# klae01/fft-conv-pytorch

Hardware: AMD Instinct MI355X
Metric: GSamples/s (output elems/s), forward fft_conv (higher is better)
Workload: dtype f32; 1 GPU; cfgA: 1D fft_conv B=32/GPU 8->8ch groups=1 spatial=[32768] kernel=[512] dilation=1 bias, fp32; tile=1024, buffer_sets=9, hip_graph=True, launches_per_graph=576, kernel_spectrum=cached per weight version (FFTConv module)

## Files before the change

### fft_conv_pytorch_amd/_native.py

```python
from __future__ import annotations

import collections
import ctypes
import os
import threading
from typing import Optional, Tuple

_HERE = os.path.dirname(os.path.abspath(__file__))
LIB_NAME = "libfftconv_amd.so"
LIB_PATH = os.environ.get("FFTCONV_LIB") or os.path.join(_HERE, LIB_NAME)

FC_OK, FC_ERR_INVALID, FC_ERR_UNSUPPORTED, FC_ERR_HIP = 0, 1, 2, 3
PAD_MODES = {"constant": 0, "zeros": 0, "reflect": 1, "replicate": 2, "circular": 3}
ABI_VERSION = 7

EXPORTS = (
    "fc_version", "fc_last_error", "fc_plan_create", "fc_plan_destroy", "fc_output_shape",
    "fc_kernel_spectrum_bytes", "fc_workspace_bytes", "fc_plan_tile", "fc_plan_layout", "fc_transform_kernel",
    "fc_forward", "fc_forward_stamped", "fc_wgrad1d_slices", "fc_wgrad1d", "fc_wgrad1d_db", "fc_wgrad1d_db_supported",
    "fc_debug_grid", "fc_wgrad_nd_plan_create", "fc_wgrad_nd", "fc_debug_route",
    "fc_long_geometry", "fc_long_plan_create", "fc_long_plan_destroy", "fc_long_plan_info", "fc_long_transform_kernel",
    "fc_long_forward", "fc_long_transform_kernel_io", "fc_long_forward_io",
    "fc_long_geometry_ext", "fc_long_plan_create_ext",
    "fc_long_geometry_kind", "fc_long_plan_create_kind", "fc_long_plan_kind",
    "fc_long_forward_lay",
    "fc_long_phases_geometry", "fc_long_phases_plan_create",
    "fc_long_decim_geometry", "fc_long_decim_plan_create",
    "fc_long_wgrad_geometry", "fc_long_wgrad_check_io", "fc_long_wgrad_plan_create", "fc_long_wgrad_plan_destroy",
    "fc_long_wgrad_plan_info", "fc_long_wgrad",
)

ROUTE_KINDS = ("f32_1d", "f32_nd", "f64_direct", "f64_fft_1d", "f64_fft_nd", "f64_fft_long")
ROUTE_WORDS = {
    "f32_1d": ("T", "ntiles", "pers_nb", "ph", "ph2", "slot_tiles", "nseg", "diag", "bd_gs", "wide", "dense",
               "chunk_launches", "accumulate", "n_ochunks", "pers_items"),
# ... 117 lines not shown
        lib.fc_wgrad1d_db.restype = i32
        lib.fc_wgrad1d_db_supported.argtypes = [ctypes.POINTER(FcDesc)]
        lib.fc_wgrad1d_db_supported.restype = i32
        lib.fc_wgrad_nd_plan_create.argtypes = [ctypes.POINTER(FcDesc), ctypes.POINTER(vp)]
        lib.fc_wgrad_nd_plan_create.restype = i32
        lib.fc_wgrad_nd.argtypes = [vp, vp, vp, vp, vp, vp, vp]
        lib.fc_wgrad_nd.restype = i32
        lib.fc_forward_stamped.argtypes = [vp, vp, vp, vp, vp, vp, vp, vp]
        lib.fc_forward_stamped.restype = i32
        lib.fc_plan_layout.argtypes = [vp, ctypes.POINTER(ctypes.c_int32 * 8)]
        lib.fc_plan_layout.restype = i32
        lib.fc_debug_grid.argtypes = [vp]
        lib.fc_debug_grid.restype = ctypes.c_longlong
        lib.fc_debug_route.argtypes = [vp, ctypes.POINTER(ctypes.c_int32 * 16)]
        lib.fc_debug_route.restype = i32
        i64x8 = ctypes.POINTER(ctypes.c_int64 * 8)
        lib.fc_long_geometry.argtypes = [ctypes.POINTER(FcLongDesc), i64x8]
        lib.fc_long_geometry.restype = i32
        lib.fc_long_plan_create.argtypes = [ctypes.POINTER(FcLongDesc), ctypes.POINTER(vp)]
        lib.fc_long_plan_create.restype = i32
        lib.fc_long_plan_destroy.argtypes = [vp]
        lib.fc_long_plan_destroy.restype = None
        lib.fc_long_plan_info.argtypes = [vp, i64x8]
        lib.fc_long_plan_info.restype = i32
        lib.fc_long_transform_kernel.argtypes = [vp, vp, vp, vp, vp]
        lib.fc_long_transform_kernel.restype = i32
        lib.fc_long_forward.argtypes = [vp, vp, vp, vp, vp, vp, vp]
        lib.fc_long_forward.restype = i32
        lib.fc_long_transform_kernel_io.argtypes = [vp, vp, i32, vp, vp, vp]
        lib.fc_long_transform_kernel_io.restype = i32
# ... 92 lines not shown

    def run(self, x_ptr: int, dy_ptr: int, dw_ptr: int, spectrum_ptr: int, workspace_ptr: Optional[int], stream: int):
        st = self._lib.fc_wgrad_nd(self._h, x_ptr, dy_ptr, dw_ptr, spectrum_ptr, workspace_ptr, stream)
        if st != FC_OK:
            _raise(self._lib, st)

    def __del__(self):
        try:
            if getattr(self, "_h", None):
                self._lib.fc_plan_destroy(self._h)
                self._h = None
        except Exception:
            pass


def read_route(lib, handle) -> dict:
    words = (ctypes.c_int32 * 16)()
    st = lib.fc_debug_route(handle, ctypes.byref(words))
    if st != FC_OK:
        _raise(lib, st)
    kind = ROUTE_KINDS[words[0]]
    route = {"kind": kind}
    route.update({name: int(words[1 + i]) for i, name in enumerate(ROUTE_WORDS[kind])})
    return route


def _raise(lib, status: int):
    msg = lib.fc_last_error().decode("utf-8", "replace")
    if status == FC_ERR_INVALID:
        raise ValueError(msg)
# ... 52 lines not shown
                workspace_ptr: Optional[int], stream: int):
        if self._stamps is not None:
            st = self._lib.fc_forward_stamped(self._h, x_ptr, w_hat_ptr, bias_ptr, y_ptr, workspace_ptr, stream,
                                              self._stamps)
        else:
            st = self._lib.fc_forward(self._h, x_ptr, w_hat_ptr, bias_ptr, y_ptr, workspace_ptr, stream)
        if st != FC_OK:
            _raise(self._lib, st)

    def debug_set_stamps(self, ptr: Optional[int]):
        self._stamps = ptr

    def debug_grid(self) -> int:
        return int(self._lib.fc_debug_grid(self._h))

    def __del__(self):
        try:
            if getattr(self, "_h", None):
                self._lib.fc_plan_destroy(self._h)
                self._h = None
        except Exception:
            pass


def long_desc(key: Tuple) -> FcLongDesc:
    if len(key) not in (11, 15, 16):
        raise ValueError(f"a long-plan key has 11 words, 15 with (pad_mode, src_up, tap_dil, out_step), or 16 with those and "
                         f"the kind of a complex plan; got {len(key)}")
    d = FcLongDesc()
    (d.batch, d.in_channels, d.out_channels, d.groups, d.length, d.kernel, d.pad_left, d.pad_right, d.out_keep,
# ... 236 lines not shown
```

### fft_conv_pytorch_amd/csrc/conv1d_pers.hpp

```cpp
#pragma once
#include "conv1d_fused.hpp"

namespace fc {

struct WorkItem {
  int b0, nbc, tile, goc;
};

struct Conv1dPersArgs {
  Conv1dArgs c;
  const WorkItem* items;
  int n_items;
};

__device__ __forceinline__ void stamp_item(unsigned long long* buf, int item, int slot) {
  if (buf != nullptr && (threadIdx.x & 63) == 0)
    buf[((size_t)item * 16 + (threadIdx.x >> 6)) * 16 + slot] = __builtin_amdgcn_s_memrealtime();
}
__device__ __forceinline__ void stamp_clock(unsigned long long* buf, int item, int slot) {
  if (buf != nullptr && (threadIdx.x & 63) == 0)
    buf[((size_t)item * 16 + (threadIdx.x >> 6)) * 16 + slot] = __builtin_amdgcn_s_memtime();
}

namespace pers {
// ... 24 lines not shown
  constexpr int T = G::T;
  constexpr int NPI = CIB / 2;
  constexpr int NSEQ = NB * NPI;
  static_assert(NT == NSEQ * G::TS, "one thread slot per point group of every sequence");
  static_assert((T / 2) % NT == 0, "bin pairs divide evenly over the threads");
  static_assert(NPI % 2 == 0, "the spectrum pipeline alternates two register sets");
  static_assert(NB * CIB * 2 <= 64, "the self-paired bins are handled by one wave");
  constexpr int BP = (T / 2) / NT;
  constexpr int TWN = P * G::N2;
  extern __shared__ __attribute__((aligned(16))) f2 lds[];
  const Conv1dArgs& a = pa.c;
  const Io<IO> io(a.io);
  constexpr unsigned ES = Io<IO>::B;
  auto stampi = [&](int item, int slot) { if constexpr (STAMPS) stamp_item(a.stamps, item, slot); };
  auto stampc = [&](int item, int slot) { if constexpr (STAMPS) stamp_clock(a.stamps, item, slot); };
  const int nph = PHASES ? a.ph : 1;

  const int tid = threadIdx.x;
  const int sq = tid / G::TS;
  const int tseq = tid % G::TS;
  static_assert(G::TS <= 64 && (NPI * G::TS) % 64 == 0, "a batch slot is a whole number of wavefronts");
  const int wv = __builtin_amdgcn_readfirstlane(tid >> 6);
  const int nb = PH4 ? ((tid >> 5) & 1) : (PH2 ? 2 * (wv / NPI) + ((tid >> 5) & 1)
               : (BPAIR ? 2 * __builtin_amdgcn_readfirstlane(tid / (CIB * G::TS)) : __builtin_amdgcn_readfirstlane(tid / (NPI * G::TS))));
  const int pr = PH4 ? wv : (PH2 ? wv % NPI : (BPAIR ? sq % CIB : sq % NPI));
  f2* twl = lds;
  f2* zbuf = lds + TWN;
  f2* zseq = PH4 ? zbuf + (nb * 8 + pr) * G::LSEQ : zbuf + (nb * NPI + pr) * G::LSEQ;

  const PadMap pm = make_padmap(a.pad_mode, a.L);
  const BufRsrc twB = make_rsrc(a.twB, (unsigned)(S * P * 8));
  const size_t wgroup = (size_t)a.Cog_pad * (a.Cig_pad / 2) * (T / 2);

  auto fetch = [&](const WorkItem& wi, f2 (&v)[P]) {
    if constexpr (BPAIR) {
      const int g = wi.goc / a.n_ochunks;
      const int bA = a.slot_tiles ? wi.b0 : wi.b0 + nb, bB = a.slot_tiles ? bA : bA + 1;
      const int tA = a.slot_tiles ? wi.tile + nb : wi.tile, tB = a.slot_tiles ? tA + 1 : tA;
      const int bfirst = wi.b0, blast = a.slot_tiles ? bfirst : wi.b0 + wi.nbc - 1;
      const int posA = tA * a.V - a.pad + (SEG ? a.pos_shift : 0), posB = tB * a.V - a.pad + (SEG ? a.pos_shift : 0);
      const bool interior = (posA >= 0) && (posA + (T - 1) < a.L) && (posB >= 0) && (posB + (T - 1) < a.L);
      const auto* xbase = io_ptr<IO>(a.x) + ((size_t)bfirst * a.Cin + (size_t)g * a.Cig) * a.L;
      const BufRsrc xg = make_rsrc(xbase, (unsigned)(((size_t)(blast - bfirst) * a.Cin + a.Cig) * a.L * ES));
      const bool hasA = nb < wi.nbc && pr < a.Cig, hasB = nb + 1 < wi.nbc && pr < a.Cig;
      const unsigned roA = ((unsigned)(bA - bfirst) * (unsigned)a.Cin + (unsigned)pr) * (unsigned)a.L * ES;
      const unsigned roB = ((unsigned)(bB - bfirst) * (unsigned)a.Cin + (unsigned)pr) * (unsigned)a.L * ES;
      if (interior && hasB) {
        const unsigned v0 = roA + (unsigned)(posA + tseq) * ES, v1 = roB + (unsigned)(posB + tseq) * ES;
#pragma unroll
        for (int n1 = 0; n1 < P; ++n1) {
          v[n1].x = io.load(xg, v0, G::N2 * n1 * ES);
          v[n1].y = io.load(xg, v1, G::N2 * n1 * ES);
        }
      } else {
#pragma unroll
        for (int n1 = 0; n1 < P; ++n1) {
          v[n1].x = io.load(xg, padded_offset<ES>(roA, posA + G::N2 * n1 + tseq, a.L, a.pad, pm, hasA), 0);
          v[n1].y = io.load(xg, padded_offset<ES>(roB, posB + G::N2 * n1 + tseq, a.L, a.pad, pm, hasB), 0);
        }
      }
      return;
    }
    const int g = wi.goc / a.n_ochunks;
    const int vb = a.slot_tiles ? wi.b0 : wi.b0 + nb;
    const int tile = a.slot_tiles ? wi.tile + nb : wi.tile;
    const int bfirst = wi.b0 / nph, blast = a.slot_tiles ? bfirst : (wi.b0 + wi.nbc - 1) / nph;
    const int b = vb / nph, phase = vb - b * nph;
    const int pos0 = tile * a.V * nph + phase - a.pad + (SEG ? a.pos_shift : 0);
    const bool interior = (pos0 >= 0) && (pos0 + (T - 1) * nph < a.L);
    const bool act_in = nb < wi.nbc;
    const auto* xbase = io_ptr<IO>(a.x) + ((size_t)bfirst * a.Cin + (size_t)g * a.Cig) * a.L;
    const BufRsrc xg = make_rsrc(xbase, (unsigned)(((size_t)(blast - bfirst) * a.Cin + a.Cig) * a.L * ES));
    const int ci0 = 2 * pr;
    const bool has0 = act_in && ci0 < a.Cig && (!DIAG || g * CIB + ci0 < a.Cin);
    const bool has1 = act_in && ci0 + 1 < a.Cig && (!DIAG || g * CIB + ci0 + 1 < a.Cin);
    const unsigned ro0 = ((unsigned)(b - bfirst) * (unsigned)a.Cin + (unsigned)ci0) * (unsigned)a.L * ES;
    const unsigned ro1 = ro0 + (unsigned)a.L * ES;
    if constexpr (PH4) {
      const int bA = wi.b0 / nph, phA = wi.b0 - bA * nph;
      const int posA = wi.tile * a.V * nph + phA - a.pad;
      const bool all_in = (posA >= 0) && (posA + 3 + (T - 1) * nph < a.L);
      const bool chan = pr < a.Cig;
      const unsigned rA = ((unsigned)(bA - bfirst) * (unsigned)a.Cin + (unsigned)pr) * (unsigned)a.L * ES;
      const bool al16 = (((size_t)xbase | ((size_t)a.L * ES) | ((size_t)(unsigned)posA * ES)) & (4 * ES - 1)) == 0;
      if (all_in && al16) {
        const unsigned q0 = chan ? rA + (unsigned)(posA + (tid & 63) * nph) * ES : 0x80000000u;
        const unsigned step4 = 64u * ES * (unsigned)nph;
#pragma unroll
        for (int m = 0; m < P / 2; ++m) {
          const f4 q = io.load4(xg, q0, step4 * m);
          v[2 * m] = q.xy; v[2 * m + 1] = q.zw;
        }
        return;
      }
      const unsigned ro = ((unsigned)(bA - bfirst) * (unsigned)a.Cin + (unsigned)pr) * (unsigned)a.L * ES;
#pragma unroll
      for (int n1 = 0; n1 < P; ++n1) {
        const int pos = posA + 2 * nb + (G::N2 * n1 + tseq) * nph;
        v[n1].x = io.load(xg, padded_offset<ES>(ro, pos, a.L, a.pad, pm, chan), 0);
        v[n1].y = io.load(xg, padded_offset<ES>(ro, pos + 1, a.L, a.pad, pm, chan), 0);
      }
      return;
    }
    if constexpr (PH2) {
      const int vbA = wi.b0 + 2 * (wv / NPI), bA = vbA / nph, phA = vbA - bA * nph;
      const int posA = wi.tile * a.V * nph + phA - a.pad;
      const bool both_in = (posA >= 0) && (posA + 1 + (T - 1) * nph < a.L);
      if (both_in && __all(has1)) {
        const unsigned rA = ((unsigned)(bA - bfirst) * (unsigned)a.Cin + (unsigned)ci0) * (unsigned)a.L * ES;
        const unsigned q0 = rA + (unsigned)(posA + (tid & 63) * nph) * ES, q1 = q0 + (unsigned)a.L * ES;
        const unsigned step2 = 64u * ES * (unsigned)nph;
#pragma unroll
        for (int m = 0; m < P / 2; ++m) {
          f2 cx = io.load2(xg, q0, step2 * m), cy = io.load2(xg, q1, step2 * m);
          v[2 * m].x = cx.x; v[2 * m + 1].x = cx.y; v[2 * m].y = cy.x; v[2 * m + 1].y = cy.y;
        }
        return;
      }
    }
    if (interior && has1 && !PHASES) {
      const unsigned v0 = ro0 + (unsigned)(pos0 + tseq) * ES, v1 = ro1 + (unsigned)(pos0 + tseq) * ES;
#if FC_DIAG == 7
#pragma unroll
      for (int n1 = 0; n1 < P; ++n1) { v[n1] = mk2(1e-3f * n1, (float)tseq); asm volatile("" : "+v"(v[n1])); }
      (void)v0; (void)v1;
      return;
#endif
#pragma unroll
      for (int n1 = 0; n1 < P; ++n1) {
        v[n1].x = io.load(xg, v0, G::N2 * n1 * ES);
        v[n1].y = io.load(xg, v1, G::N2 * n1 * ES);
      }
    } else if (interior && has1) {
      const unsigned v0 = ro0 + (unsigned)(pos0 + tseq * nph) * ES, v1 = ro1 + (unsigned)(pos0 + tseq * nph) * ES;
      const unsigned step = (unsigned)(G::N2 * ES) * (unsigned)nph;
#pragma unroll
      for (int n1 = 0; n1 < P; ++n1) {
        v[n1].x = io.load(xg, v0, step * n1);
        v[n1].y = io.load(xg, v1, step * n1);
      }
    } else {
#pragma unroll
      for (int n1 = 0; n1 < P; ++n1) {
        const int pos = pos0 + (G::N2 * n1 + tseq) * nph;
        v[n1].x = io.load(xg, padded_offset<ES>(ro0, pos, a.L, a.pad, pm, has0), 0);
        v[n1].y = io.load(xg, padded_offset<ES>(ro1, pos, a.L, a.pad, pm, has1), 0);
      }
    }
  };

  auto fetch_finish = [&](const WorkItem& wi, f2 (&v)[P]) {
    if constexpr (PH4) {
      const int bA = wi.b0 / nph, phA = wi.b0 - bA * nph;
      const int posA = wi.tile * a.V * nph + phA - a.pad;
      const int bfirst = wi.b0 / nph;
      const auto* xbase = io_ptr<IO>(a.x) + ((size_t)bfirst * a.Cin + (size_t)(wi.goc / a.n_ochunks) * a.Cig) * a.L;
      const bool all_in = (posA >= 0) && (posA + 3 + (T - 1) * nph < a.L);
      const bool al16 = (((size_t)xbase | ((size_t)a.L * ES) | ((size_t)(unsigned)posA * ES)) & (4 * ES - 1)) == 0;
      if (all_in && al16) {
#pragma unroll
        for (int m = 0; m < P / 2; ++m) { swap_halves_c<0>(v[2 * m], v[2 * m + 1]); swap_halves_c<1>(v[2 * m], v[2 * m + 1]); }
      }
    }
    if constexpr (PH2) {
      const bool has1 = nb < wi.nbc && 2 * pr + 1 < a.Cig;
      const int vbA = wi.b0 + 2 * (wv / NPI), bA = vbA / nph, phA = vbA - bA * nph;
      const int posA = wi.tile * a.V * nph + phA - a.pad;
      const bool both_in = (posA >= 0) && (posA + 1 + (T - 1) * nph < a.L);
      if (both_in && __all(has1)) {
#pragma unroll
        for (int m = 0; m < P / 2; ++m) { swap_halves_c<0>(v[2 * m], v[2 * m + 1]); swap_halves_c<1>(v[2 * m], v[2 * m + 1]); }
      }
    }
  };

  auto run = [&](const WorkItem& wi, int it, f2 (&v)[P], bool more, const WorkItem& wnext, f2 (&vnext)[P]) {
    const int g = wi.goc / a.n_ochunks, oc = wi.goc % a.n_ochunks;
    const bool act_in = PH4 ? true : nb < wi.nbc;
    const BufRsrc wg = DIAG ? make_rsrc(a.wspec + (size_t)g * NPI * (T / 2), (unsigned)(NPI * (T / 2) * 16))
                            : make_rsrc(a.wspec + (size_t)g * wgroup, (unsigned)(wgroup * 16));
    stampi(it, 0);
    stampc(it, 12);
    const int cg0 = g * a.Cog + oc * a.cob + ((PH4 || BPAIR) ? pr : 2 * pr);
    const bool ok0 = !DIAG || cg0 < a.Cout, ok1 = !BPAIR && (!DIAG || cg0 + 1 < a.Cout);
    const BufRsrc brs = make_rsrc(a.bias, a.bias ? (unsigned)a.Cout * 4u : 0u);
    float bias0 = buf_load_f32(brs, ok0 ? (unsigned)cg0 * 4u : 0xFFFFFFFFu, 0);
    float bias1 = BPAIR ? 0.f : buf_load_f32(brs, ok1 ? (unsigned)(cg0 + 1) * 4u : 0xFFFFFFFFu, 0);
    if (STAMPS && a.stamps) { asm volatile("s_waitcnt vmcnt(0)" ::: "memory"); stampi(it, 1); }
    if (act_in) {
      fetch_finish(wi, v);
      passA_fft_twiddle_store_lds<G, -1>(v, zseq, tseq, twl);
      stampi(it, 2);
// ... 342 lines not shown
#pragma unroll
        for (int p = 0; p < NPI; ++p) {
          acc = fmaf(2.f * sbz[p].x, (tid & 1) ? sbw[p].y : sbw[p].x, acc);
          acc = fmaf(2.f * sbz[p].y, (tid & 1) ? sbw[p].w : sbw[p].z, acc);
        }
        float* dstf = reinterpret_cast<float*>(zbuf + (sb_b * NPI + (sb_o >> 1)) * G::LSEQ + G::nat(sb_f)) + (sb_o & 1);
        *dstf = acc;
      }
    }
    }
    stampi(it, 6);
#if FC_DIAG != 5
    __syncthreads();
#endif
    stampi(it, 7);
    asm volatile("" : "+v"(bias0), "+v"(bias1));
    if (more) fetch(wnext, vnext);
    if (act_in) {
      nat_load<G>(v, zseq, tseq);
      seq_sync<G>();
      passA_fft_twiddle_store_lds<G, +1>(v, zseq, tseq, twl);
      stampi(it, 8);
      seq_sync<G>();
      stampi(it, 9);
      passB_load<G>(v, zseq, tseq);
      const int j = passB_compute<G, +1>(v, tseq, twB);
      if (more) {
#pragma unroll
        for (int n1 = 0; n1 < P; ++n1) asm volatile("" : "+v"(vnext[n1]));
      }
      const int o1 = tseq >> G::LGS;
// ... 165 lines not shown
                io.store(v[2 * m + 1].y + bias1, yr, (w1 + ES) | dB, step2 * m);
              }
            });
          }
        });
      } else {
        const int ystep = P * nph;
#pragma unroll
        for (int k = 0; k < P; ++k)
          if (nbase + P * k < limit) { y0[ystep * k] = io.out(v[k].x + bias0); y1[ystep * k] = io.out(v[k].y + bias1); }
      }
    }
    stampi(it, 10);
    if (STAMPS && a.stamps) { asm volatile("s_waitcnt vmcnt(0)" ::: "memory"); stampi(it, 11); stampc(it, 13); }
    seq_sync<G>();
  };

  const int it0 = blockIdx.x, it1 = blockIdx.x + gridDim.x;
  const bool two = it1 < pa.n_items;
  const WorkItem w0 = pa.items[it0];
  const WorkItem w1 = pa.items[two ? it1 : it0];
  f2 va[P], vb[P];
  fetch(w0, va);
  copy_table_to_lds<TWN, NT>(twl, a.twA, tid);
  __syncthreads();
  run(w0, it0, va, two, w1, vb);
  if (two) run(w1, it1, vb, false, w1, va);
}

}
```

### fft_conv_pytorch_amd/csrc/fc_api.cpp

```cpp
#include <hip/hip_runtime.h>

#include <cmath>
#include <cstdarg>
#include <cstdio>
#include <cstdlib>
#include <cstring>
#include <map>
#include <memory>
#include <mutex>
#include <string>
#include <vector>

#include "fc_plan.h"

namespace {

thread_local std::string g_err;
std::mutex g_tw_mutex;
std::map<std::pair<int, int>, fc::Twiddles> g_tw;

}

namespace fc {

// ... 291 lines not shown
  switch (p.kind) {
    case PlanKind::F32_1D:
      if (p.f1d.pers_nb) return (long long)p.f1d.pers_items * 16;
      return (long long)p.d.batch * p.ntiles * p.n_ochunks * p.G;
    case PlanKind::F32_ND:
      if (p.fnd.planes) {
        const long long ncol = p.fnd.planes == 1 ? (long long)fc::kPlCols * p.fnd.nxt * p.fnd.nyt : p.fnd.Fxt;
        return (long long)p.d.batch * p.ntiles * (p.fnd.Cog_pad / p.fnd.cob) * p.d.groups * ((ncol / 16 + 7) / 8) * 8;
      } else {
        const long long ncol = p.nd == 2 ? p.fnd.Fxt : (long long)p.fnd.Fxt * p.fnd.tm->T * p.fnd.nyt;
        return (long long)p.d.batch * p.ntiles * (p.fnd.Cog_pad / p.fnd.cob) * p.d.groups * ((ncol + 7) / 8) * 8;
      }
    default:
      return 0;
  }
}

int fc_debug_route(const fc_plan* plan, int32_t route[16]) {
  if (!plan || !route) return fail(FC_ERR_INVALID, "null argument");
  const fc_plan& p = *plan;
  for (int i = 0; i < 16; ++i) route[i] = 0;
  route[0] = (int32_t)p.kind;
  switch (p.kind) {
    case PlanKind::F32_1D: {
      const int32_t w[] = {p.tile->T, p.ntiles, p.f1d.pers_nb, p.f1d.ph, p.f1d.ph2, p.f1d.slot_tiles, p.f1d.nseg,
                           p.f1d.diag, p.f1d.bd_gs, p.f1d.wide, p.f1d.dense, p.f1d.chunk_launches, p.accumulate,
                           p.n_ochunks, p.f1d.pers_items};
      for (int i = 0; i < 15; ++i) route[1 + i] = w[i];
      break;
    }
// ... 106 lines not shown
```

### fft_conv_pytorch_amd/csrc/fc_plan.h

```cpp
#pragma once
#include <hip/hip_runtime.h>

#include <cstdint>
#include <cstring>

#include "fc_internal.h"
#include "fftconv_amd.h"

namespace fc {

int fail(int code, const char* fmt, ...);

#define FC_HIP(expr)                                                                         \
  do {                                                                                       \
    hipError_t e_ = (expr);                                                                  \
    if (e_ != hipSuccess) return ::fc::fail(FC_ERR_HIP, "%s: %s", #expr, hipGetErrorString(e_)); \
  } while (0)

#define FC_HIP_SETUP(expr)                                                               \
  do {                                                                                   \
    hipError_t e_ = (expr);                                                              \
    if (e_ != hipSuccess) {                                                              \
      const char* name_ = hipGetErrorName(e_);                                           \
      (void)hipGetLastError();                                                           \
// ... 5 lines not shown
    }                                                                                    \
  } while (0)

const TileImpl* const* all_tiles(int* n);
const TileImpl* find_tile(int T);

struct Twiddles {
  f2* twA = nullptr;
  f2* twB = nullptr;
};
int get_twiddles(const TileImpl* t, Twiddles* out);
int find_twiddles(const TileImpl* t, Twiddles* out);

int current_device_cus(int* cus_out);
int64_t round_up(int64_t v, int64_t m);

enum class PlanKind {
  F32_1D,
  F32_ND,
  F64_DIRECT,
  F64_FFT_1D,
  F64_FFT_ND,
  F64_FFT_LONG,
};

}

struct fc_plan {
  fc_desc d;
  fc::PlanKind kind;
// ... 93 lines not shown
```

### fft_conv_pytorch_amd/csrc/fft_engine.hpp

```cpp
#pragma once
#include <hip/hip_runtime.h>
#include <type_traits>

#ifndef FC_DIAG
#define FC_DIAG 0
#endif

namespace fc {

typedef float f2 __attribute__((ext_vector_type(2)));
typedef float f4 __attribute__((ext_vector_type(4)));

__device__ __forceinline__ f2 pkfma(f2 a, f2 b, f2 c) { return __builtin_elementwise_fma(a, b, c); }
__device__ __forceinline__ f2 mk2(float x, float y) { f2 r; r.x = x; r.y = y; return r; }
__device__ __forceinline__ f2 add_mi(f2 a, f2 b) {
  f2 d; asm("v_pk_add_f32 %0, %1, %2 op_sel:[0,1] op_sel_hi:[1,0] neg_hi:[0,1]" : "=v"(d) : "v"(a), "v"(b)); return d;
}
__device__ __forceinline__ f2 add_pi(f2 a, f2 b) {
  f2 d; asm("v_pk_add_f32 %0, %1, %2 op_sel:[0,1] op_sel_hi:[1,0] neg_lo:[0,1]" : "=v"(d) : "v"(a), "v"(b)); return d;
}
__device__ __forceinline__ f2 add_conj(f2 a, f2 b) {
  f2 d; asm("v_pk_add_f32 %0, %1, %2 neg_hi:[0,1]" : "=v"(d) : "v"(a), "v"(b)); return d;
}
__device__ __forceinline__ f2 sub_conj_divi(f2 a, f2 b) {
// ... 217 lines not shown
constexpr int IO_F32 = 0, IO_H16 = 1;
constexpr int IO_CODE_F16 = 2, IO_CODE_BF16 = 3;
constexpr bool io_is_h16(int code) { return code == IO_CODE_F16 || code == IO_CODE_BF16; }
template <int IO>
struct Io;
template <>
struct Io<IO_F32> {
  using T = float;
  static constexpr unsigned B = 4;
  __device__ __forceinline__ explicit Io(int) {}
  __device__ __forceinline__ float in(float v) const { return v; }
  __device__ __forceinline__ float out(float v) const { return v; }
  __device__ __forceinline__ float load(BufRsrc r, unsigned voff, unsigned soff) const { return buf_load_f32(r, voff, soff); }
  __device__ __forceinline__ f2 load2(BufRsrc r, unsigned voff, unsigned soff) const { return buf_load_f32x2(r, voff, soff); }
  __device__ __forceinline__ f4 load4(BufRsrc r, unsigned voff, unsigned soff) const { return buf_load_f32x4(r, voff, soff); }
  __device__ __forceinline__ void store(float v, BufRsrc r, unsigned voff, unsigned soff) const { buf_store_f32(v, r, voff, soff); }
  __device__ __forceinline__ void store2(f2 v, BufRsrc r, unsigned voff, unsigned soff) const { buf_store_f32x2(v, r, voff, soff); }
  __device__ __forceinline__ void store4(f4 v, BufRsrc r, unsigned voff, unsigned soff) const {
    u32x4 d;
    d.x = __float_as_uint(v.x); d.y = __float_as_uint(v.y); d.z = __float_as_uint(v.z); d.w = __float_as_uint(v.w);
    __builtin_amdgcn_raw_buffer_store_b128(d, r, voff, soff, 0);
  }
};
template <>
struct Io<IO_H16> {
  using T = unsigned short;
  static constexpr unsigned B = 2;
  bool bf;
  __device__ __forceinline__ explicit Io(int code) : bf(code == IO_CODE_BF16) {}
  __device__ __forceinline__ float in(unsigned h) const {
// ... 7 lines not shown
  }
  __device__ __forceinline__ unsigned pack(float lo, float hi) const {
    const bf16x2 b = {(__bf16)lo, (__bf16)hi};
    const f16x2 h = {(_Float16)lo, (_Float16)hi};
    return bf ? __builtin_bit_cast(unsigned, b) : __builtin_bit_cast(unsigned, h);
  }
  __device__ __forceinline__ float load(BufRsrc r, unsigned voff, unsigned soff) const {
    return in(__builtin_amdgcn_raw_buffer_load_b16(r, voff, soff, 0));
  }
  __device__ __forceinline__ f2 load2(BufRsrc r, unsigned voff, unsigned soff) const {
    const unsigned w = __builtin_amdgcn_raw_buffer_load_b32(r, voff, soff, 0);
    return mk2(in(w), in(w >> 16));
  }
  __device__ __forceinline__ f4 load4(BufRsrc r, unsigned voff, unsigned soff) const {
    const u32x2 w = __builtin_amdgcn_raw_buffer_load_b64(r, voff, soff, 0);
    f4 o; o.x = in(w.x); o.y = in(w.x >> 16); o.z = in(w.y); o.w = in(w.y >> 16);
    return o;
  }
  __device__ __forceinline__ void store(float v, BufRsrc r, unsigned voff, unsigned soff) const {
    __builtin_amdgcn_raw_buffer_store_b16(out(v), r, voff, soff, 0);
  }
  __device__ __forceinline__ void store2(f2 v, BufRsrc r, unsigned voff, unsigned soff) const {
    __builtin_amdgcn_raw_buffer_store_b32(pack(v.x, v.y), r, voff, soff, 0);
  }
  __device__ __forceinline__ void store4(f4 v, BufRsrc r, unsigned voff, unsigned soff) const {
    u32x2 d; d.x = pack(v.x, v.y); d.y = pack(v.z, v.w);
    __builtin_amdgcn_raw_buffer_store_b64(d, r, voff, soff, 0);
  }
};
template <int IO>
// ... 220 lines not shown
```

### fft_conv_pytorch_amd/csrc/host_1d.cpp

```cpp
#include <hip/hip_runtime.h>

#include <algorithm>
#include <cmath>
#include <cstdlib>
#include <vector>

#include "fc_plan.h"

namespace fc {

static bool fast_path_eligible(const fc_plan* p) {
  const fc_desc& d = p->d;
  if (p->CB != 8 || p->accumulate || p->f1d.chunk_launches || p->Cog % 8 != 0 || d.stride[0] != 1) return false;
  if (((int64_t)d.in_channels * 3 + p->Cig) * d.spatial[0] * 4 >= ((int64_t)1 << 32)) return false;
  if ((int64_t)p->cob * p->out_sp[0] * 4 >= 0x7F000000LL) return false;
  return true;
}

static int choose_fast_path(fc_plan* p, int* tile_out) {
  const fc_desc& d = p->d;
  const char* env = getenv("FFTCONV_PERS");
  const int want = env ? atoi(env) : -1;
  const bool fast_ok = want != 0 && fast_path_eligible(p);
  int cus = 256;
// ... 16 lines not shown
      if ((round || p->f1d.diag) && c.nb == 0) continue;
      if (c.T < Kd || p->accumulate) continue;
      if (c.nb != 0 && !fast_ok) continue;
      if (want > 0 && c.nb != want) continue;
      const int64_t V = c.T - Kd + 1;
      if (V * 4 < c.T) continue;
      const int64_t nt = (Lfull + V - 1) / V;
      const bool by_tiles = c.nb > B;
      if (by_tiles && nt < c.nb) continue;
      const int64_t groups_of = by_tiles ? B * ((nt + c.nb - 1) / c.nb) : ((B + std::max(c.nb, 1) - 1) / std::max(c.nb, 1)) * nt;
      const int64_t items = groups_of * per_item_units;
      const int64_t slots = (int64_t)cus * c.wgs_per_cu;
      double est;
      if (c.nb == 0) {
        est = (double)((items + slots - 1) / slots) * c.t_item;
      } else {
        const int64_t grid = std::max<int64_t>((items + 1) / 2, std::min<int64_t>(items, slots));
        const double ipw = (double)items / (double)grid;
        auto t_occ = [&](int64_t wgs) {
          const int64_t occ = std::min<int64_t>(c.wgs_per_cu, (wgs + cus - 1) / cus);
          return c.wgs_per_cu > 1 ? c.t_alone + (c.t_item - c.t_alone) * (double)(occ - 1) / (double)(c.wgs_per_cu - 1) : c.t_item;
        };
        const int64_t full = grid / slots, rem = grid % slots;
        est = kLaunchUs + (double)full * std::ceil(ipw) * c.t_item + (rem ? std::ceil(ipw) * t_occ(rem) : 0.0);
      }
      if (best_T == 0 || est < best) { best = est; best_T = c.T; best_nb = c.nb; best_ph = ph; best_tiles = by_tiles; }
    }
  }
  if (best_T == 0) return FC_OK;
  *tile_out = best_T;
  p->f1d.pers_nb_choice = best_nb;
  p->f1d.ph = best_ph;
// ... 49 lines not shown
          for (int t0 = 0; t0 < p->ntiles; t0 += nb) {
            const int n = std::min(nb, p->ntiles - t0);
            bool border = false;
            for (int k = 0; k < n; ++k) border |= is_border(t0 + k);
            if ((pass == 0) == border) items.push_back({(int)vb, n, t0, goc});
          }
  } else {
  for (int tile : tile_order)
    for (int goc = 0; goc < p->n_ochunks * p->G; ++goc)
      for (int c = 0; c < nfull; ++c) items.push_back({c * nb, nb, tile, goc});
  }
  const char* ph_env = getenv("FFTCONV_PH2");
  const int ph_want = ph_env ? atoi(ph_env) : 2;
  const bool ph_base = p->f1d.ph > 1 && !p->f1d.slot_tiles && !p->f1d.diag && !p->f1d.wide && p->f1d.nseg == 1 && nb >= 2 && t->S == 1;
  const bool quads = ph_want >= 2 && ph_base && p->f1d.ph % 4 == 0 && nb == 4 && p->Cig == 8 && p->cob == 8 && p->Cog % 8 == 0 && !p->f1d.bd_gs;
  if (nb >= 2 && (int64_t)items.size() > slots && !quads) {
    const int64_t tail = (int64_t)items.size() % slots;
    if (tail > 0 && tail <= slots / 2) {
      std::vector<fc::WorkItem> split;
      for (int64_t k = (int64_t)items.size() - tail; k < (int64_t)items.size(); ++k) {
        const fc::WorkItem w = items[k];
        const int h = w.nbc / 2;
        if (h == 0) { split.push_back(w); continue; }
        split.push_back({w.b0, h, w.tile, w.goc});
        if (p->f1d.slot_tiles) split.push_back({w.b0, w.nbc - h, w.tile + h, w.goc});
        else split.push_back({w.b0 + h, w.nbc - h, w.tile, w.goc});
      }
      items.resize(items.size() - tail);
      items.insert(items.end(), split.begin(), split.end());
    }
  }
  if (rem && !p->f1d.slot_tiles)
    for (int tile = 0; tile < p->ntiles; ++tile)
      for (int goc = 0; goc < p->n_ochunks * p->G; ++goc) items.push_back({nfull * nb, rem, tile, goc});
  if (items.size() > 0x7fffffffu) return FC_OK;
  p->f1d.pers_items = (int)items.size();
  p->f1d.pers_grid = (int)std::max<int64_t>((p->f1d.pers_items + 1) / 2, std::min<int64_t>(p->f1d.pers_items, slots));
  if (p->f1d.wide) p->f1d.pers_grid = p->f1d.pers_items;
  FC_HIP_SETUP(hipMalloc(&p->f1d.d_items, items.size() * sizeof(fc::WorkItem)));
  FC_HIP_SETUP(hipMemcpy(p->f1d.d_items, items.data(), items.size() * sizeof(fc::WorkItem), hipMemcpyHostToDevice));
  p->f1d.pers_nb = nb;
  p->f1d.ph2 = quads ? 2 : ((ph_want != 0 && ph_base && p->f1d.ph % 2 == 0) ? 1 : 0);
  return FC_OK;
}

static int plan_1d_inner(fc_plan* p) {
  const fc_desc& d = p->d;
  p->f1d.nseg = 1; p->f1d.seg_taps = (int)d.kernel[0]; p->f1d.kd_plan = p->kd[0];
  {
    const bool sharing_shape = p->CB == 8 && p->Cog % 8 == 0 && d.stride[0] == 1;
    const bool want_seg = p->kd[0] > 4096 || (sharing_shape && p->kd[0] > 1537 && !d.tile_hint);
    if (want_seg) {
// ... 391 lines not shown
```

### include/fftconv_amd.h

```cpp
#ifndef FFTCONV_AMD_H
#define FFTCONV_AMD_H

#include <stddef.h>
#include <stdint.h>

#ifdef __cplusplus
extern "C" {
#endif

#define FC_ABI_VERSION 7

enum fc_status {
  FC_OK = 0,
  FC_ERR_INVALID = 1,
  FC_ERR_UNSUPPORTED = 2,
  FC_ERR_HIP = 3
};

enum fc_pad_mode { FC_PAD_CONSTANT = 0, FC_PAD_REFLECT = 1, FC_PAD_REPLICATE = 2, FC_PAD_CIRCULAR = 3 };
enum fc_dtype {
  FC_F32 = 0,
  FC_F64 = 1,
  FC_F16 = 2,
  FC_BF16 = 3,
// ... 46 lines not shown
int fc_wgrad1d_slices(const fc_desc* desc);
int fc_wgrad1d(const fc_desc* desc, const float* x, const float* dy, float* partial, int slices, void* hip_stream);
int fc_wgrad1d_db_supported(const fc_desc* desc);
int fc_wgrad1d_db(const fc_desc* desc, const float* x, const float* dy, float* partial, float* db_partial,
                  long long slice_stride, int slices, void* hip_stream);

int fc_wgrad_nd_plan_create(const fc_desc* conv_desc, fc_plan** out_plan);
int fc_wgrad_nd(const fc_plan* plan, const float* x, const float* dy, float* dw, void* spectrum, void* workspace,
                void* hip_stream);

int fc_forward_stamped(const fc_plan* plan, const float* x, const void* w_hat, const float* bias, float* y,
                       void* workspace, void* hip_stream, void* stamps);
long long fc_debug_grid(const fc_plan* plan);

int fc_debug_route(const fc_plan* plan, int32_t route[16]);

typedef struct fc_long_desc {
  int64_t batch, in_channels, out_channels, groups;
  int64_t length;
  int64_t kernel;
  int64_t pad_left, pad_right;
  int64_t out_keep;
  int32_t flip;
  int32_t has_bias;
} fc_long_desc;

typedef struct fc_long_plan fc_long_plan;

enum { FC_LONG_INFO_WORDS = 8 };

// ... 87 lines not shown
```

Baseline: 263.4 GSamples/s.

## Make persistent 1D conv kernel loop over arbitrary work items with prefetched descriptors

The persistent forward kernel used to handle at most two work items per workgroup, which forced a grid of at least half the item count. It now loops over items with a stride of the grid size, prefetching the item after next through a buffer load and double-buffering signal fetches, so the grid can be capped at the slot count when items exceed twice the slots. Raw loads are split from widening so all loads are issued before conversion, and the cost model adds a launch term for the many-items case. An env override for the grid and debug entry points are added. The added loop state and per-iteration register pinning may raise register pressure.

```diff
diff --git a/fft_conv_pytorch_amd/_native.py b/fft_conv_pytorch_amd/_native.py
--- a/fft_conv_pytorch_amd/_native.py
+++ b/fft_conv_pytorch_amd/_native.py
@@ -18,7 +18,7 @@
     "fc_version", "fc_last_error", "fc_plan_create", "fc_plan_destroy", "fc_output_shape",
     "fc_kernel_spectrum_bytes", "fc_workspace_bytes", "fc_plan_tile", "fc_plan_layout", "fc_transform_kernel",
     "fc_forward", "fc_forward_stamped", "fc_wgrad1d_slices", "fc_wgrad1d", "fc_wgrad1d_db", "fc_wgrad1d_db_supported",
-    "fc_debug_grid", "fc_wgrad_nd_plan_create", "fc_wgrad_nd", "fc_debug_route",
+    "fc_debug_grid", "fc_wgrad_nd_plan_create", "fc_wgrad_nd", "fc_debug_route", "fc_debug_pers_grid", "fc_debug_pers_schedule",
     "fc_long_geometry", "fc_long_plan_create", "fc_long_plan_destroy", "fc_long_plan_info", "fc_long_transform_kernel",
     "fc_long_forward", "fc_long_transform_kernel_io", "fc_long_forward_io",
     "fc_long_geometry_ext", "fc_long_plan_create_ext",
@@ -166,6 +166,10 @@
         lib.fc_debug_grid.restype = ctypes.c_longlong
         lib.fc_debug_route.argtypes = [vp, ctypes.POINTER(ctypes.c_int32 * 16)]
         lib.fc_debug_route.restype = i32
+        lib.fc_debug_pers_grid.argtypes = [vp]
+        lib.fc_debug_pers_grid.restype = ctypes.c_longlong
+        lib.fc_debug_pers_schedule.argtypes = [ctypes.c_longlong] * 4 + [i32, ctypes.POINTER(ctypes.c_longlong * 3)]
+        lib.fc_debug_pers_schedule.restype = i32
         i64x8 = ctypes.POINTER(ctypes.c_int64 * 8)
         lib.fc_long_geometry.argtypes = [ctypes.POINTER(FcLongDesc), i64x8]
         lib.fc_long_geometry.restype = i32
@@ -288,6 +292,15 @@
             pass
 
 
+def pers_schedule(full_items: int, rem_items: int, slots: int, forced_grid: int = 0, splittable: bool = True):
+    lib = load_library()
+    out = (ctypes.c_longlong * 3)()
+    st = lib.fc_debug_pers_schedule(full_items, rem_items, slots, forced_grid, int(splittable), ctypes.byref(out))
+    if st != FC_OK:
+        _raise(lib, st)
+    return tuple(int(v) for v in out)
+
+
 def read_route(lib, handle) -> dict:
     words = (ctypes.c_int32 * 16)()
     st = lib.fc_debug_route(handle, ctypes.byref(words))
@@ -370,6 +383,9 @@
     def debug_grid(self) -> int:
         return int(self._lib.fc_debug_grid(self._h))
 
+    def pers_grid(self) -> int:
+        return int(self._lib.fc_debug_pers_grid(self._h))
+
     def __del__(self):
         try:
             if getattr(self, "_h", None):
diff --git a/fft_conv_pytorch_amd/csrc/conv1d_pers.hpp b/fft_conv_pytorch_amd/csrc/conv1d_pers.hpp
--- a/fft_conv_pytorch_amd/csrc/conv1d_pers.hpp
+++ b/fft_conv_pytorch_amd/csrc/conv1d_pers.hpp
@@ -62,25 +62,36 @@
   constexpr unsigned ES = Io<IO>::B;
   auto stampi = [&](int item, int slot) { if constexpr (STAMPS) stamp_item(a.stamps, item, slot); };
   auto stampc = [&](int item, int slot) { if constexpr (STAMPS) stamp_clock(a.stamps, item, slot); };
-  const int nph = PHASES ? a.ph : 1;
-
-  const int tid = threadIdx.x;
-  const int sq = tid / G::TS;
-  const int tseq = tid % G::TS;
+  int nph = PHASES ? a.ph : 1;
+
+  int tid = threadIdx.x;
+  int sq, tseq;
   static_assert(G::TS <= 64 && (NPI * G::TS) % 64 == 0, "a batch slot is a whole number of wavefronts");
-  const int wv = __builtin_amdgcn_readfirstlane(tid >> 6);
-  const int nb = PH4 ? ((tid >> 5) & 1) : (PH2 ? 2 * (wv / NPI) + ((tid >> 5) & 1)
-               : (BPAIR ? 2 * __builtin_amdgcn_readfirstlane(tid / (CIB * G::TS)) : __builtin_amdgcn_readfirstlane(tid / (NPI * G::TS))));
-  const int pr = PH4 ? wv : (PH2 ? wv % NPI : (BPAIR ? sq % CIB : sq % NPI));
+  int wv, nb, pr;
+  f2* zbuf = lds + TWN;
+  f2* zseq;
+  auto place = [&]() {
+    sq = tid / G::TS;
+    tseq = tid % G::TS;
+    wv = __builtin_amdgcn_readfirstlane(tid >> 6);
+    nb = PH4 ? ((tid >> 5) & 1) : (PH2 ? 2 * (wv / NPI) + ((tid >> 5) & 1)
+       : (BPAIR ? 2 * __builtin_amdgcn_readfirstlane(tid / (CIB * G::TS)) : __builtin_amdgcn_readfirstlane(tid / (NPI * G::TS))));
+    pr = PH4 ? wv : (PH2 ? wv % NPI : (BPAIR ? sq % CIB : sq % NPI));
+    zseq = PH4 ? zbuf + (nb * 8 + pr) * G::LSEQ : zbuf + (nb * NPI + pr) * G::LSEQ;
+  };
+  place();
   f2* twl = lds;
-  f2* zbuf = lds + TWN;
-  f2* zseq = PH4 ? zbuf + (nb * 8 + pr) * G::LSEQ : zbuf + (nb * NPI + pr) * G::LSEQ;
 
   const PadMap pm = make_padmap(a.pad_mode, a.L);
   const BufRsrc twB = make_rsrc(a.twB, (unsigned)(S * P * 8));
   const size_t wgroup = (size_t)a.Cog_pad * (a.Cig_pad / 2) * (T / 2);
 
   auto fetch = [&](const WorkItem& wi, f2 (&v)[P]) {
+    typename Io<IO>::R rx[P], ry[P];
+    auto widen_all = [&]() {
+#pragma unroll
+      for (int n1 = 0; n1 < P; ++n1) v[n1] = mk2(io.widen(rx[n1]), io.widen(ry[n1]));
+    };
     if constexpr (BPAIR) {
       const int g = wi.goc / a.n_ochunks;
       const int bA = a.slot_tiles ? wi.b0 : wi.b0 + nb, bB = a.slot_tiles ? bA : bA + 1;
@@ -96,16 +107,15 @@
       if (interior && hasB) {
         const unsigned v0 = roA + (unsigned)(posA + tseq) * ES, v1 = roB + (unsigned)(posB + tseq) * ES;
 #pragma unroll
+        for (int n1 = 0; n1 < P; ++n1) { rx[n1] = io.load_raw(xg, v0, G::N2 * n1 * ES); ry[n1] = io.load_raw(xg, v1, G::N2 * n1 * ES); }
+        widen_all();
+      } else {
+#pragma unroll
         for (int n1 = 0; n1 < P; ++n1) {
-          v[n1].x = io.load(xg, v0, G::N2 * n1 * ES);
-          v[n1].y = io.load(xg, v1, G::N2 * n1 * ES);
-        }
-      } else {
-#pragma unroll
-        for (int n1 = 0; n1 < P; ++n1) {
-          v[n1].x = io.load(xg, padded_offset<ES>(roA, posA + G::N2 * n1 + tseq, a.L, a.pad, pm, hasA), 0);
-          v[n1].y = io.load(xg, padded_offset<ES>(roB, posB + G::N2 * n1 + tseq, a.L, a.pad, pm, hasB), 0);
-        }
+          rx[n1] = io.load_raw(xg, padded_offset<ES>(roA, posA + G::N2 * n1 + tseq, a.L, a.pad, pm, hasA), 0);
+          ry[n1] = io.load_raw(xg, padded_offset<ES>(roB, posB + G::N2 * n1 + tseq, a.L, a.pad, pm, hasB), 0);
+        }
+        widen_all();
       }
       return;
     }
@@ -134,9 +144,12 @@
       if (all_in && al16) {
         const unsigned q0 = chan ? rA + (unsigned)(posA + (tid & 63) * nph) * ES : 0x80000000u;
         const unsigned step4 = 64u * ES * (unsigned)nph;
+        typename Io<IO>::R4 rq[P / 2];
+#pragma unroll
+        for (int m = 0; m < P / 2; ++m) rq[m] = io.load4_raw(xg, q0, step4 * m);
 #pragma unroll
         for (int m = 0; m < P / 2; ++m) {
-          const f4 q = io.load4(xg, q0, step4 * m);
+          const f4 q = io.widen4(rq[m]);
           v[2 * m] = q.xy; v[2 * m + 1] = q.zw;
         }
         return;
@@ -145,9 +158,10 @@
 #pragma unroll
       for (int n1 = 0; n1 < P; ++n1) {
         const int pos = posA + 2 * nb + (G::N2 * n1 + tseq) * nph;
-        v[n1].x = io.load(xg, padded_offset<ES>(ro, pos, a.L, a.pad, pm, chan), 0);
-        v[n1].y = io.load(xg, padded_offset<ES>(ro, pos + 1, a.L, a.pad, pm, chan), 0);
-      }
+        rx[n1] = io.load_raw(xg, padded_offset<ES>(ro, pos, a.L, a.pad, pm, chan), 0);
+        ry[n1] = io.load_raw(xg, padded_offset<ES>(ro, pos + 1, a.L, a.pad, pm, chan), 0);
+      }
+      widen_all();
       return;
     }
     if constexpr (PH2) {
@@ -158,9 +172,12 @@
         const unsigned rA = ((unsigned)(bA - bfirst) * (unsigned)a.Cin + (unsigned)ci0) * (unsigned)a.L * ES;
         const unsigned q0 = rA + (unsigned)(posA + (tid & 63) * nph) * ES, q1 = q0 + (unsigned)a.L * ES;
         const unsigned step2 = 64u * ES * (unsigned)nph;
+        typename Io<IO>::R2 rcx[P / 2], rcy[P / 2];
+#pragma unroll
+        for (int m = 0; m < P / 2; ++m) { rcx[m] = io.load2_raw(xg, q0, step2 * m); rcy[m] = io.load2_raw(xg, q1, step2 * m); }
 #pragma unroll
         for (int m = 0; m < P / 2; ++m) {
-          f2 cx = io.load2(xg, q0, step2 * m), cy = io.load2(xg, q1, step2 * m);
+          const f2 cx = io.widen2(rcx[m]), cy = io.widen2(rcy[m]);
           v[2 * m].x = cx.x; v[2 * m + 1].x = cx.y; v[2 * m].y = cy.x; v[2 * m + 1].y = cy.y;
         }
         return;
@@ -175,25 +192,22 @@
       return;
 #endif
 #pragma unroll
-      for (int n1 = 0; n1 < P; ++n1) {
-        v[n1].x = io.load(xg, v0, G::N2 * n1 * ES);
-        v[n1].y = io.load(xg, v1, G::N2 * n1 * ES);
-      }
+      for (int n1 = 0; n1 < P; ++n1) { rx[n1] = io.load_raw(xg, v0, G::N2 * n1 * ES); ry[n1] = io.load_raw(xg, v1, G::N2 * n1 * ES); }
+      widen_all();
     } else if (interior && has1) {
       const unsigned v0 = ro0 + (unsigned)(pos0 + tseq * nph) * ES, v1 = ro1 + (unsigned)(pos0 + tseq * nph) * ES;
       const unsigned step = (unsigned)(G::N2 * ES) * (unsigned)nph;
 #pragma unroll
-      for (int n1 = 0; n1 < P; ++n1) {
-        v[n1].x = io.load(xg, v0, step * n1);
-        v[n1].y = io.load(xg, v1, step * n1);
-      }
+      for (int n1 = 0; n1 < P; ++n1) { rx[n1] = io.load_raw(xg, v0, step * n1); ry[n1] = io.load_raw(xg, v1, step * n1); }
+      widen_all();
     } else {
 #pragma unroll
       for (int n1 = 0; n1 < P; ++n1) {
         const int pos = pos0 + (G::N2 * n1 + tseq) * nph;
-        v[n1].x = io.load(xg, padded_offset<ES>(ro0, pos, a.L, a.pad, pm, has0), 0);
-        v[n1].y = io.load(xg, padded_offset<ES>(ro1, pos, a.L, a.pad, pm, has1), 0);
-      }
+        rx[n1] = io.load_raw(xg, padded_offset<ES>(ro0, pos, a.L, a.pad, pm, has0), 0);
+        ry[n1] = io.load_raw(xg, padded_offset<ES>(ro1, pos, a.L, a.pad, pm, has1), 0);
+      }
+      widen_all();
     }
   };
 
@@ -222,8 +236,12 @@
     }
   };
 
-  auto run = [&](const WorkItem& wi, int it, f2 (&v)[P], bool more, const WorkItem& wnext, f2 (&vnext)[P]) {
+  auto run = [&](const WorkItem& wi, int it, f2 (&v)[P], bool more, const WorkItem& wnext, f2 (&vnext)[P], int it2, WorkItem& wnn) {
+    asm volatile("" : "+v"(tid));
+    place();
+    if constexpr (PHASES) asm volatile("" : "+s"(nph));
     const int g = wi.goc / a.n_ochunks, oc = wi.goc % a.n_ochunks;
+    f4 rec = buf_load_f32x4(make_rsrc(pa.items + it2, (unsigned)sizeof(WorkItem)), 0u, 0);
     const bool act_in = PH4 ? true : nb < wi.nbc;
     const BufRsrc wg = DIAG ? make_rsrc(a.wspec + (size_t)g * NPI * (T / 2), (unsigned)(NPI * (T / 2) * 16))
                             : make_rsrc(a.wspec + (size_t)g * wgroup, (unsigned)(wgroup * 16));
@@ -596,7 +614,13 @@
     __syncthreads();
 #endif
     stampi(it, 7);
-    asm volatile("" : "+v"(bias0), "+v"(bias1));
+    asm volatile("" : "+v"(bias0), "+v"(bias1), "+v"(rec));
+    wnn.b0 = __builtin_amdgcn_readfirstlane((int)__float_as_uint(rec.x));
+    wnn.nbc = __builtin_amdgcn_readfirstlane((int)__float_as_uint(rec.y));
+    wnn.tile = __builtin_amdgcn_readfirstlane((int)__float_as_uint(rec.z));
+    wnn.goc = __builtin_amdgcn_readfirstlane((int)__float_as_uint(rec.w));
+#pragma unroll
+    for (int n1 = 0; n1 < P; ++n1) asm volatile("" : "=v"(vnext[n1]));
     if (more) fetch(wnext, vnext);
     if (act_in) {
       nat_load<G>(v, zseq, tseq);
@@ -792,18 +816,32 @@
     stampi(it, 10);
     if (STAMPS && a.stamps) { asm volatile("s_waitcnt vmcnt(0)" ::: "memory"); stampi(it, 11); stampc(it, 13); }
     seq_sync<G>();
+#pragma unroll
+    for (int n1 = 0; n1 < P; ++n1) asm volatile("" : "=v"(v[n1]));
   };
 
-  const int it0 = blockIdx.x, it1 = blockIdx.x + gridDim.x;
-  const bool two = it1 < pa.n_items;
-  const WorkItem w0 = pa.items[it0];
-  const WorkItem w1 = pa.items[two ? it1 : it0];
+  const int grid = (int)gridDim.x, n = pa.n_items;
+  int it = blockIdx.x;
+  bool moreA = n - it > grid;
+  WorkItem wa = pa.items[it];
+  WorkItem wb = pa.items[moreA ? it + grid : it];
   f2 va[P], vb[P];
-  fetch(w0, va);
+  fetch(wa, va);
   copy_table_to_lds<TWN, NT>(twl, a.twA, tid);
   __syncthreads();
-  run(w0, it0, va, two, w1, vb);
-  if (two) run(w1, it1, vb, false, w1, va);
+  for (;;) {
+    WorkItem wn;
+    const bool moreB = moreA && n - it - grid > grid;
+    run(wa, it, va, moreA, wb, vb, moreB ? it + 2 * grid : it, wn);
+    if (!moreA) break;
+    it += grid;
+    wa = wn;
+    moreA = moreB && n - it - grid > grid;
+    run(wb, it, vb, moreB, wa, va, moreA ? it + 2 * grid : it, wn);
+    if (!moreB) break;
+    it += grid;
+    wb = wn;
+  }
 }
 
 }
diff --git a/fft_conv_pytorch_amd/csrc/fc_api.cpp b/fft_conv_pytorch_amd/csrc/fc_api.cpp
--- a/fft_conv_pytorch_amd/csrc/fc_api.cpp
+++ b/fft_conv_pytorch_amd/csrc/fc_api.cpp
@@ -329,6 +329,20 @@
     default:
       return 0;
   }
+}
+
+long long fc_debug_pers_grid(const fc_plan* plan) {
+  if (!plan || plan->kind != PlanKind::F32_1D || !plan->f1d.pers_nb) return 0;
+  return plan->f1d.pers_grid;
+}
+
+int fc_debug_pers_schedule(long long full_items, long long rem_items, long long slots, long long forced_grid,
+                           int splittable, long long sched[3]) {
+  if (!sched || full_items < 0 || rem_items < 0 || slots < 1 || forced_grid < 0) return fail(FC_ERR_INVALID, "invalid argument");
+  const int64_t split = fc::pers_tail_split(full_items, slots, forced_grid, splittable != 0);
+  const int64_t items = full_items + split + rem_items;
+  sched[0] = split; sched[1] = items; sched[2] = fc::pers_grid_for(items, slots, forced_grid);
+  return FC_OK;
 }
 
 int fc_debug_route(const fc_plan* plan, int32_t route[16]) {
diff --git a/fft_conv_pytorch_amd/csrc/fc_plan.h b/fft_conv_pytorch_amd/csrc/fc_plan.h
--- a/fft_conv_pytorch_amd/csrc/fc_plan.h
+++ b/fft_conv_pytorch_amd/csrc/fc_plan.h
@@ -43,6 +43,18 @@
 
 int current_device_cus(int* cus_out);
 int64_t round_up(int64_t v, int64_t m);
+
+inline int64_t pers_grid_for(int64_t items, int64_t slots, int64_t forced) {
+  if (forced > 0) return forced < items ? forced : (items > 0 ? items : 1);
+  if (items <= 2 * slots) { const int64_t h = (items + 1) / 2, m = items < slots ? items : slots; return h > m ? h : m; }
+  return slots;
+}
+inline int64_t pers_tail_split(int64_t full_items, int64_t slots, int64_t forced, bool splittable) {
+  const int64_t round = forced > 0 ? forced : slots;
+  if (!splittable || full_items <= round) return 0;
+  const int64_t tail = full_items % round;
+  return (tail > 0 && tail <= round / 2) ? tail : 0;
+}
 
 enum class PlanKind {
   F32_1D,
diff --git a/fft_conv_pytorch_amd/csrc/fft_engine.hpp b/fft_conv_pytorch_amd/csrc/fft_engine.hpp
--- a/fft_conv_pytorch_amd/csrc/fft_engine.hpp
+++ b/fft_conv_pytorch_amd/csrc/fft_engine.hpp
@@ -255,6 +255,13 @@
   __device__ __forceinline__ float load(BufRsrc r, unsigned voff, unsigned soff) const { return buf_load_f32(r, voff, soff); }
   __device__ __forceinline__ f2 load2(BufRsrc r, unsigned voff, unsigned soff) const { return buf_load_f32x2(r, voff, soff); }
   __device__ __forceinline__ f4 load4(BufRsrc r, unsigned voff, unsigned soff) const { return buf_load_f32x4(r, voff, soff); }
+  using R = float; using R2 = f2; using R4 = f4;
+  __device__ __forceinline__ R load_raw(BufRsrc r, unsigned voff, unsigned soff) const { return buf_load_f32(r, voff, soff); }
+  __device__ __forceinline__ R2 load2_raw(BufRsrc r, unsigned voff, unsigned soff) const { return buf_load_f32x2(r, voff, soff); }
+  __device__ __forceinline__ R4 load4_raw(BufRsrc r, unsigned voff, unsigned soff) const { return buf_load_f32x4(r, voff, soff); }
+  __device__ __forceinline__ float widen(R v) const { return v; }
+  __device__ __forceinline__ f2 widen2(R2 v) const { return v; }
+  __device__ __forceinline__ f4 widen4(R4 v) const { return v; }
   __device__ __forceinline__ void store(float v, BufRsrc r, unsigned voff, unsigned soff) const { buf_store_f32(v, r, voff, soff); }
   __device__ __forceinline__ void store2(f2 v, BufRsrc r, unsigned voff, unsigned soff) const { buf_store_f32x2(v, r, voff, soff); }
   __device__ __forceinline__ void store4(f4 v, BufRsrc r, unsigned voff, unsigned soff) const {
@@ -292,6 +299,16 @@
   }
   __device__ __forceinline__ f4 load4(BufRsrc r, unsigned voff, unsigned soff) const {
     const u32x2 w = __builtin_amdgcn_raw_buffer_load_b64(r, voff, soff, 0);
+    f4 o; o.x = in(w.x); o.y = in(w.x >> 16); o.z = in(w.y); o.w = in(w.y >> 16);
+    return o;
+  }
+  using R = unsigned short; using R2 = unsigned; using R4 = u32x2;
+  __device__ __forceinline__ R load_raw(BufRsrc r, unsigned voff, unsigned soff) const { return __builtin_amdgcn_raw_buffer_load_b16(r, voff, soff, 0); }
+  __device__ __forceinline__ R2 load2_raw(BufRsrc r, unsigned voff, unsigned soff) const { return __builtin_amdgcn_raw_buffer_load_b32(r, voff, soff, 0); }
+  __device__ __forceinline__ R4 load4_raw(BufRsrc r, unsigned voff, unsigned soff) const { return __builtin_amdgcn_raw_buffer_load_b64(r, voff, soff, 0); }
+  __device__ __forceinline__ float widen(R h) const { return in(h); }
+  __device__ __forceinline__ f2 widen2(R2 w) const { return mk2(in(w), in(w >> 16)); }
+  __device__ __forceinline__ f4 widen4(R4 w) const {
     f4 o; o.x = in(w.x); o.y = in(w.x >> 16); o.z = in(w.y); o.w = in(w.y >> 16);
     return o;
   }
diff --git a/fft_conv_pytorch_amd/csrc/host_1d.cpp b/fft_conv_pytorch_amd/csrc/host_1d.cpp
--- a/fft_conv_pytorch_amd/csrc/host_1d.cpp
+++ b/fft_conv_pytorch_amd/csrc/host_1d.cpp
@@ -54,8 +54,10 @@
       double est;
       if (c.nb == 0) {
         est = (double)((items + slots - 1) / slots) * c.t_item;
+      } else if (items > 2 * slots) {
+        est = kLaunchUs + (double)((items + slots - 1) / slots) * c.t_item;
       } else {
-        const int64_t grid = std::max<int64_t>((items + 1) / 2, std::min<int64_t>(items, slots));
+        const int64_t grid = fc::pers_grid_for(items, slots, 0);
         const double ipw = (double)items / (double)grid;
         auto t_occ = [&](int64_t wgs) {
           const int64_t occ = std::min<int64_t>(c.wgs_per_cu, (wgs + cus - 1) / cus);
@@ -135,28 +137,27 @@
   const int ph_want = ph_env ? atoi(ph_env) : 2;
   const bool ph_base = p->f1d.ph > 1 && !p->f1d.slot_tiles && !p->f1d.diag && !p->f1d.wide && p->f1d.nseg == 1 && nb >= 2 && t->S == 1;
   const bool quads = ph_want >= 2 && ph_base && p->f1d.ph % 4 == 0 && nb == 4 && p->Cig == 8 && p->cob == 8 && p->Cog % 8 == 0 && !p->f1d.bd_gs;
-  if (nb >= 2 && (int64_t)items.size() > slots && !quads) {
-    const int64_t tail = (int64_t)items.size() % slots;
-    if (tail > 0 && tail <= slots / 2) {
-      std::vector<fc::WorkItem> split;
-      for (int64_t k = (int64_t)items.size() - tail; k < (int64_t)items.size(); ++k) {
-        const fc::WorkItem w = items[k];
-        const int h = w.nbc / 2;
-        if (h == 0) { split.push_back(w); continue; }
-        split.push_back({w.b0, h, w.tile, w.goc});
-        if (p->f1d.slot_tiles) split.push_back({w.b0, w.nbc - h, w.tile + h, w.goc});
-        else split.push_back({w.b0 + h, w.nbc - h, w.tile, w.goc});
-      }
-      items.resize(items.size() - tail);
-      items.insert(items.end(), split.begin(), split.end());
-    }
+  const char* grid_env = getenv("FFTCONV_PERS_GRID");
+  const int64_t forced_grid = (grid_env && !p->f1d.wide) ? std::max<int64_t>(0, atoll(grid_env)) : 0;
+  if (const int64_t tail = fc::pers_tail_split((int64_t)items.size(), slots, forced_grid, nb >= 2 && !quads)) {
+    std::vector<fc::WorkItem> split;
+    for (int64_t k = (int64_t)items.size() - tail; k < (int64_t)items.size(); ++k) {
+      const fc::WorkItem w = items[k];
+      const int h = w.nbc / 2;
+      if (h == 0) { split.push_back(w); continue; }
+      split.push_back({w.b0, h, w.tile, w.goc});
+      if (p->f1d.slot_tiles) split.push_back({w.b0, w.nbc - h, w.tile + h, w.goc});
+      else split.push_back({w.b0 + h, w.nbc - h, w.tile, w.goc});
+    }
+    items.resize(items.size() - tail);
+    items.insert(items.end(), split.begin(), split.end());
   }
   if (rem && !p->f1d.slot_tiles)
     for (int tile = 0; tile < p->ntiles; ++tile)
       for (int goc = 0; goc < p->n_ochunks * p->G; ++goc) items.push_back({nfull * nb, rem, tile, goc});
   if (items.size() > 0x7fffffffu) return FC_OK;
   p->f1d.pers_items = (int)items.size();
-  p->f1d.pers_grid = (int)std::max<int64_t>((p->f1d.pers_items + 1) / 2, std::min<int64_t>(p->f1d.pers_items, slots));
+  p->f1d.pers_grid = (int)fc::pers_grid_for(p->f1d.pers_items, slots, forced_grid);
   if (p->f1d.wide) p->f1d.pers_grid = p->f1d.pers_items;
   FC_HIP_SETUP(hipMalloc(&p->f1d.d_items, items.size() * sizeof(fc::WorkItem)));
   FC_HIP_SETUP(hipMemcpy(p->f1d.d_items, items.data(), items.size() * sizeof(fc::WorkItem), hipMemcpyHostToDevice));
diff --git a/include/fftconv_amd.h b/include/fftconv_amd.h
--- a/include/fftconv_amd.h
+++ b/include/fftconv_amd.h
@@ -84,6 +84,11 @@
 long long fc_debug_grid(const fc_plan* plan);
 
 int fc_debug_route(const fc_plan* plan, int32_t route[16]);
+
+long long fc_debug_pers_grid(const fc_plan* plan);
+
+int fc_debug_pers_schedule(long long full_items, long long rem_items, long long slots, long long forced_grid,
+                           int splittable, long long sched[3]);
 
 typedef struct fc_long_desc {
   int64_t batch, in_channels, out_channels, groups;
```

After: 259.1 GSamples/s. 0.984x the previous value.
